# Pixel-Talk/CanonSwap

Measured on AMD Instinct MI355X. Metric: frames/sec at 512x512 (generator hot path F->W->T->R->W->G), higher is better.
Workload: dtype f16; 1 GPU; BASELINE configs[2]: 512x512 video, 64 frames batched per launch on each GPU, steady state over 1280 frames (20 launches per GPU) (256x256 crops in, random-init weights of the real architecture); frames_per_launch_per_gpu=64, frames_total=1280, parallelism=frame-shard x1, identities_resident=1, latency_mode=False, accumulate=fp32, debug_decodes=False

## Files before the change

canonswap_amd/csrc/common.h:

```cpp
#pragma once
#include <hip/hip_runtime.h>
#include <stdint.h>

typedef _Float16 half_t;
typedef _Float16 h8_t __attribute__((ext_vector_type(8)));
typedef _Float16 h4_t __attribute__((ext_vector_type(4)));
typedef float f4_t __attribute__((ext_vector_type(4)));

enum { ACT_NONE = 0, ACT_RELU = 1, ACT_LRELU = 2, ACT_SIGMOID = 3, ACT_GELU = 4 };
enum { MODE_STD = 0, MODE_TBLEND = 1, MODE_SPADE = 2, MODE_PIXSHUF = 3,
       MODE_STDSTAT = 4 };
enum { CFG_128x128 = 0, CFG_128x64 = 1, CFG_256x32 = 2, CFG_256x16 = 3 };
enum { CFG_H_128x128 = 10, CFG_H_128x64 = 11, CFG_H_256x32 = 12, CFG_H_128x32 = 13, CFG_H_128x16 = 14, CFG_H_256x16 = 15,
       CFG_H_SK128x32 = 16 , CFG_H_128x256 = 17,
       CFG_H_128x160 = 18 ,
       CFG_H_256x160 = 19 ,
       CFG_H_256x64 = 20 ,
       CFG_VOL32 = 30 , CFG_WIDE = 31 ,
       CFG_LAT = 32  };

struct TDesc {
    void* p;
    long sN, sD, sH, sW;
};
// ... 45 lines not shown
    int ep_general;
    int pool_hw;
    int spmul;
    const half_t* xs_w; TDesc xs_res, xs_out; int xs_cout;
    int persist_total;
    unsigned in_sample_bytes;
    int nphase;
    long ph_wofs[4];
    unsigned ph_ooff[4];
    int ph_PH[4], ph_PW[4];
    int xf_kind;
    int v32_srows;
    TDesc xf_y, xf_res, xf_out;
    const float* xf_stats; const float* xf_gamma; const float* xf_beta;
    float xf_slope;
#ifdef CS_TIMELINE
    unsigned long long* tl;
    long tl_cap;
#endif
};

__device__ __forceinline__ float gn_scale(float rstd, float gamma) { return rstd * gamma; }
__device__ __forceinline__ float gn_shift(float mean, float sc, float beta) { return fmaf(-mean, sc, beta); }
__device__ __forceinline__ float gn_lrelu(float v, float sc, float sh, float rr, float slope)
{
    float a = fmaf(v, sc, sh);
    a = a + rr;
    return fmaxf(a, a * slope);
}

// ... 15 lines not shown
    long sN, sH, sW;
    const half_t* w1; const half_t* w2;
    const float* b1; const float* b2; const float* s2; const float* t2;
    int act1; float slope1;
    int N, H, W;
};
bool vol32_fused_supported(const ResBlock3dCall& c);
int launch_vol32_fused(const ResBlock3dCall& c, hipStream_t st);
bool vol32_supported(const ConvParams& p);
int vol32_stat_nblk(const ConvParams& p);
int launch_vol32(const ConvParams& p, hipStream_t st);
bool conv_wide_supported(const ConvParams& p, int mode);
int launch_conv_wide(const ConvParams& p, int mode, hipStream_t st);
bool conv_lat_supported(const ConvParams& p, int mode);
int launch_conv_lat(const ConvParams& p, int mode, hipStream_t st);
const half_t* cs_zero_page();

int launch_conv_first(const float* img, const float* w, const float* b, half_t* out, int N, int H, int W, hipStream_t st);
int launch_avgpool(const half_t* in, int N, int D, int H, int W, int C, TDesc out, hipStream_t st);
int launch_dm_compress(const float* f, const float* w, const float* b, half_t* comp, int N, int D, int H, int W, hipStream_t st);
int launch_dm_sparse(const half_t* comp, const float* kp_d, const float* kp_s, half_t* out, int out_stride, int N, int D,
                     int H, int W, hipStream_t st, bool shared_comp = false, bool shared_kps = false);
int launch_dm_softmax(const float* part, const float* bias, const float* kp_d, const float* kp_s, float* deform, float* mask_out,
                      int N, int D, int H, int W, hipStream_t st, int compact = 0, bool shared_kps = false);
int launch_dm_softmax_warp(const float* part, const float* bias, const float* kp_d, const float* kp_s, const float* in, float* out32,
                           half_t* out16, float* deform, int N, int D, int H, int W, hipStream_t st, int compact = 0, bool shared_in = false,
                           bool shared_kps = false);
int launch_occ_finish(const float* part, float bias, float* occ, int N, int H, int W, hipStream_t st);
int launch_occ_finish49(const float* part, float bias, float* occ, int N, int H, int W, hipStream_t st);
int launch_grid_sample(const float* in, const float* grid, float* out32, half_t* out16, int N, int D, int H, int W, hipStream_t st,
// ... 45 lines not shown
```

canonswap_amd/csrc/conv_epilogue.h:

```cpp
#pragma once
#include "common.h"

#ifndef EP_TL
#define EP_TL(i) do { } while (0)
#endif
typedef unsigned int ep_u4_t __attribute__((ext_vector_type(4)));
typedef unsigned int ep_u2_t __attribute__((ext_vector_type(2)));

static inline int ep_check_extents(const ConvParams& p, const char* who)
{
    auto span = [&](const TDesc& t) -> long {
        return (long)(p.N - 1) * t.sN + (long)(p.D - 1) * t.sD + (long)(p.H - 1) * t.sH + (long)(p.W - 1) * t.sW + p.Cout;
    };
    auto wide = [&](const TDesc& t) { return t.sD >= (1L << 23) || t.sH >= (1L << 23) || t.sW >= (1L << 23); };
    const long lim = 1L << 31;
    long ph_max = 0;
    for (int z = 0; z < p.nphase && z < 4; ++z) ph_max = p.ph_ooff[z] > ph_max ? (long)p.ph_ooff[z] : ph_max;
    if ((p.out0.p && span(p.out0) + ph_max >= lim) || (p.out1.p && span(p.out1) >= lim) || (p.res.p && span(p.res) >= lim)) {
        cs_set_error("%s: a tensor of this launch spans 2^31 elements or more (32-bit in-tensor offsets)", who);
        return -1;
    }
    if ((p.out0.p && wide(p.out0)) || (p.out1.p && wide(p.out1)) || (p.res.p && wide(p.res)) || p.D >= (1 << 22) || p.H >= (1 << 22) ||
        p.W >= (1 << 22)) {
        cs_set_error("%s: an axis stride of 2^23 elements or more (24-bit multiplies in the addressing)", who);
// ... 155 lines not shown
            float ep_pa[4], ep_pb[4]; \
_Pragma("unroll") \
            for (int r = 0; r < 4; ++r) { \
                ep_pa[r] = ep_row_sum16(ep_sum[EP_STAT ? ci : 0][r]); ep_pb[r] = ep_row_sum16(ep_sq[EP_STAT ? ci : 0][r]); \
                ep_sum[EP_STAT ? ci : 0][r] = 0.f; ep_sq[EP_STAT ? ci : 0][r] = 0.f; \
            } \
             \
            if (l15 == 0 && cb < p.Cout) { \
                float4* dst = (float4*)(p.stat_out + (((long)tn * ep_nblk + ep_blk) * p.Cout + cb) * 2); \
                dst[0] = make_float4(ep_pa[0], ep_pb[0], ep_pa[1], ep_pb[1]); \
                dst[1] = make_float4(ep_pa[2], ep_pb[2], ep_pa[3], ep_pb[3]); \
            } \
        } \
    }

#ifndef EP_GSEL_V
#define EP_GSEL_V 0
#endif
#ifndef EP_BLK_V
#define EP_BLK_V(sg) ((tile_lin % ep_tiles) * (BM / (EP_SG * 16)) + ep_wpx * (EP_WPX / EP_SG) + (sg))
#define EP_NBLK_V (ep_tiles * (BM / (EP_SG * 16)))
#endif
#ifndef EP_SLICE_FENCE
#define EP_SLICE_FENCE
#endif
#ifndef EP_FG
#define EP_FG 8
#endif
#ifndef EP_FG_F32
#define EP_FG_F32 4
// ... 19 lines not shown
#define EP_O1ONLY_V 0
#endif
#ifndef EP_MLIN_V
#define EP_MLIN_V 0
#endif
#ifndef EP_DUP_V
#define EP_DUP_V 0
#endif
#define EP_SPMULB 256
#define EP_GELUB 512
#define EP_FETCH_ROUND(PG0, BI) \
    if (EP_PF && !EP_EARLY && (ep_fetch || ep_has_ps)) { \
_Pragma("unroll") \
        for (int g = 0; g < EP_G; ++g) { \
            int bw, bh, bd, bn; \
            { int t = (ep_wpx * EP_WPX + (PG0) + g) << 4; bw = t & mW; t >>= lgTW; bh = t & mH; t >>= lgTH; bd = t & mD; t >>= lgTD; bn = t; } \
            if (!EPFAST && ep_nb + ep_ln + bn >= p.N) continue; \
            if (ep_has_ps) ep_ps2[BI][g] = p.pixscale[ep_lane_ps + (unsigned)((((bn * p.D + bd) * p.H + bh) * p.W + bw) * p.ps_stride)]; \
            if (ep_fetch) { \
                const unsigned xb = ep_lane_res + (unsigned)(bn * (int)p.res.sN + bd * (int)p.res.sD + (bh >> ep_rs) * (int)p.res.sH + \
                                                            (bw >> ep_rs) * (int)p.res.sW); \
_Pragma("unroll") \
                for (int ci = 0; ci < WCH; ci += CSTEP) { \
                    const int cb = ep_chan(EP_PAIR, CSTEP, n0 + wch * WCH * 16, ci, l4); \
                    if (!EPALL && cb >= p.Cout) continue; \
                    if (ep_res32) ep_raw2[BI][g][(EP_PF ? ci / CSTEP : 0)] = *(const ep_u4_t*)((const float*)p.res.p + (xb + (unsigned)cb)); \
                    else if (ep_mr && ep_second(EP_PAIR, ci)) {  } \
                    else if (ep_mr && (EPALL || cb + 4 < p.Cout)) ep_raw2[BI][g][(EP_PF ? ci / CSTEP : 0)] = *(const ep_u4_t*)((const half_t*)p.res.p + (xb + (unsigned)cb)); \
                    else { \
                        const ep_u2_t q2 = *(const ep_u2_t*)((const half_t*)p.res.p + (xb + (unsigned)cb)); \
                        ep_raw2[BI][g][(EP_PF ? ci / CSTEP : 0)][0] = q2[0]; ep_raw2[BI][g][(EP_PF ? ci / CSTEP : 0)][1] = q2[1]; \
// ... 79 lines not shown
    ep_u4_t ep_raw2[EP_PIPE ? 2 : 1][EP_G][EP_NCI]; float ep_ps2[EP_PIPE ? 2 : 1][EP_G]; \
    if (EP_PIPE) { EP_FETCH_ROUND(0, 0) } \
_Pragma("unroll") \
    for (int pg = 0; pg < EP_WPX; pg += EP_G) { \
    const int ep_bi = EP_PIPE ? ((pg / EP_G) & 1) : 0; \
    if (!EP_PIPE) { EP_FETCH_ROUND(pg, 0) } \
    else if (pg + EP_G < EP_WPX) { EP_FETCH_ROUND(pg + EP_G, EP_PIPE ? (((pg / EP_G) + 1) & 1) : 0) } \
    ep_u4_t (&ep_raw)[EP_G][EP_NCI] = ep_raw2[ep_bi]; float (&ep_ps)[EP_G] = ep_ps2[ep_bi]; \
    if (pg == 0) EP_TL(6); \
_Pragma("unroll") \
    for (int g = 0; g < EP_G; ++g) { \
        const int pi = pg + g; \
        if (pi == 1) EP_TL(7); \
        if (pi > 0 && pi % EP_SG == 0) { EP_STAT_FLUSH(pi / EP_SG - 1) } \
        int bw, bh, bd, bn; \
        { int t = (ep_wpx * EP_WPX + pi) << 4; bw = t & mW; t >>= lgTW; bh = t & mH; t >>= lgTH; bd = t & mD; t >>= lgTD; bn = t; } \
        if (!EPFAST && ep_nb + ep_ln + bn >= p.N) continue; \
        float ps = 1.f; \
        if (ep_has_ps) ps = EP_PF ? ep_ps[g] : p.pixscale[ep_lane_ps + (unsigned)((((bn * p.D + bd) * p.H + bh) * p.W + bw) * p.ps_stride)]; \
        const unsigned xb = ep_lane_res + (unsigned)(bn * (int)p.res.sN + bd * (int)p.res.sD + (bh >> ep_rs) * (int)p.res.sH + (bw >> ep_rs) * (int)p.res.sW); \
        const unsigned ob0 = ep_lane_o0 + (unsigned)(bn * (int)p.out0.sN + bd * (int)p.out0.sD + (bh >> EP_PS) * (int)p.out0.sH + (bw >> EP_PS) * (int)p.out0.sW); \
        const unsigned ob1 = ep_lane_o1 + (unsigned)(bn * (int)p.out1.sN + bd * (int)p.out1.sD + bh * (int)p.out1.sH + bw * (int)p.out1.sW); \
        float ep_vh[4] = {0.f, 0.f, 0.f, 0.f}, ep_uh[4] = {0.f, 0.f, 0.f, 0.f};       \
_Pragma("unroll") \
        for (int ci = 0; ci < WCH; ci += CSTEP) { \
            const int cb = ep_chan(EP_PAIR, CSTEP, n0 + wch * WCH * 16, ci, l4); \
            if (!EPALL && cb >= p.Cout) continue; \
            float rr[4] = {0.f, 0.f, 0.f, 0.f};      \
            if (ep_has_res) { \
                if (EP_EARLY) { \
                    const h4_t hx = __builtin_bit_cast(h4_t, ep_xpre[EP_EARLY ? pi : 0][EP_EARLY ? ci / 2 : 0]); \
// ... 173 lines not shown
```

canonswap_amd/csrc/conv_halo_kernel.h:

```cpp
#pragma once
#include <type_traits>
#include <utility>
#include <cstdlib>
#include "common.h"
#ifdef CS_TIMELINE
#define EP_TL(i) TL_STAMP(i)
#endif
#define EP_POOL_WSH_V EP_POOL_WSH_K
#define EP_POOL_HSH_V EP_POOL_HSH_K
#define EP_SPMUL_V EP_SPMUL_K
#define EP_DUP_V EP_DUP_K
#define EP_MLIN_V EP_MLIN_K
#define EP_O1ONLY_V EP_O1ONLY_K
#define EP_O0_EXTRA_V ep_o0_extra
#include "conv_epilogue.h"

typedef unsigned int u4_t __attribute__((ext_vector_type(4)));
__device__ __forceinline__ unsigned mdiv(unsigned u, unsigned magic) { return magic ? __umulhi(u, magic) : u; }

template <int OFF>
__device__ __forceinline__ void wfrag_load(u4_t& dst, const half_t* ptr)
{
    asm volatile("global_load_dwordx4 %0, %1, off offset:%2" : "=v"(dst) : "v"(ptr), "n"(OFF));
}
template <int N>
__device__ __forceinline__ void wait_vmcnt_le()
{
    asm volatile("s_waitcnt vmcnt(%0)" ::"n"(N) : "memory");
}
// ... 45 lines not shown
    if (PAD == 2) return ST == 3 ? 16 : (ST == 9 ? 19 : ((ST == 7 || ST == 8) ? 15 : (ST == 16 ? 13 : 8)));
    return ST == 4 ? 18 : ((ST == 3 || ST == 7 || ST == 8 || ST == 9) ? 13 : (ST == 12 ? 9 : 8));
}
template <int ST, int PAD> __host__ __device__ constexpr int halo_lane_pos(int l)
{
#ifdef CS_LDS_V1
    return l;
#else
    using SS = StaticShape<ST>;
    if (ST == 0 || SS::KW != 3 || SS::LW > 3 || SS::LW < 2) return l;
    if (SS::LW == 2 && PAD == 2) return ((l & 1) << 1) | ((l & 2) << 2) | ((l >> 2) & 1) | ((l & 8) >> 1);
    return ((l & 1) << 1) | ((l & 2) << 1) | ((l >> 2) & 1) | (l & 8);
#endif
}

template <class F, int... I> __device__ __forceinline__ void halo_static_for_impl(F&& f, std::integer_sequence<int, I...>) { (f(std::integral_constant<int, I>{}), ...); }
template <int N, class F> __device__ __forceinline__ void halo_static_for(F&& f) { halo_static_for_impl(static_cast<F&&>(f), std::make_integer_sequence<int, N>{}); }

template <int WCH, int PFS, int HI, int ST0>
constexpr int halo_ring_young(int st, int L, int NP, bool dma_cur)
{
    auto dma = [&](int u, bool on) { return (on && u >= ST0 && u < ST0 + HI) ? 1 : 0; };
    auto cur_before = [&](int from_step ) {
        int n = 0;
        for (int u = from_step; u < st; ++u) n += (u >= 1 ? WCH : 0) + dma(u, dma_cur);
        return n;
    };
    if (st >= PFS) {
        const int u0 = st - PFS + 1;
        return dma(u0, dma_cur) + cur_before(u0 + 1);
// ... 35 lines not shown
    constexpr int SLP = SL + PAD;
    constexpr bool EP_POOLK = ST != 0 && !SK && MODE == MODE_STD && WCH == 2 && SS::KD == 3 && SS::KH == 3 && SS::KW == 3 && (SS::LW == 3 || SS::LW == 2) && SS::LH >= 1;
    constexpr bool EP_POOLK2 = halo_pool2d<CK, WPX, WCH, WVP, MODE, SK, ST>();
    constexpr bool XSK = ST == 1 && !SK && MODE == MODE_STD && CK == 64 && WCH == 4 && WPX == 8 && WVP == 1;
#ifdef CS_NO_SPMUL_FAST
    constexpr bool EP_SPMUL_K = false;
#else
    constexpr bool EP_SPMUL_K = ST == 1 && !SK && MODE == MODE_STD && CK == 64 && WCH == 4 && WPX == 8 && WVP == 1;
#endif
    constexpr bool EP_O1ONLY_K = ST == 16 && !SK && MODE == MODE_STD;
    constexpr bool EP_MLIN_K = ST == 15 && !SK && MODE == MODE_STD;
    constexpr bool EP_DUP_K = (ST == 11 || ST == 14 || ST == 15) && !SK && MODE == MODE_STD && WCH == 2 && WPX == 8;
    constexpr int EP_POOL_WSH_K = EP_POOLK ? halo_pool_shift<ST, PAD>(0) : (EP_POOLK2 ? 1 : 0);
    constexpr int EP_POOL_HSH_K = EP_POOLK ? halo_pool_shift<ST, PAD>(SS::LW) : 0;
    constexpr int VS = SLP * 16;
    constexpr int HI = halo_hi<ST, PAD>();
    constexpr int KH32 = CK / 32;
    constexpr int PFD = 4;
    constexpr int SKS = SK ? 4 : 1;
    static_assert(WVP * WVC == 4, "4 waves per workgroup");
    static_assert(!SK || (WVC == 1 && WPX == 8), "split-K variants: every wave covers all 128 positions");

    extern __shared__ __attribute__((aligned(16))) unsigned char smem[];
#ifdef CS_TIMELINE
    unsigned long long tl_t[8] = {0, 0, 0, 0, 0, 0, 0, 0};
    const unsigned long long tl_real0 = __builtin_amdgcn_s_memrealtime();
    TL_STAMP(0);
#endif

#ifdef CS_DEPHASE
// ... 124 lines not shown
            for (int q0 = 0; q0 < nitems; q0 += 256) {
                const int q = q0 + tid;
                if (q < nitems) {
                    bool inb;
                    const int o = piece_off(q, inb);
                    const bool ok = inb && ((q % SLP) * 8 < climit);
                    glds(ok ? p.in + o + coff : p.zero, buf, q0 + wave * 64);
                }
            }
        }
    };

    int abase[WPX];
#pragma unroll
    for (int pi = 0; pi < WPX; ++pi) {
        int m = wpx * WPX * 16 + pi * 16 + l15p;
        const int wl = m & mW; m >>= lgTW;
        const int hl = m & mH; m >>= lgTH;
        const int dl = m & mD; m >>= lgTD;
        abase[pi] = (((m * HD + dl) * HH + hl) * HW + wl) * VS + l4 * 16;
    }
    const int nck = (p.Cin + CK - 1) / CK;
    const int j0 = SK ? wave : 0;
    int cc_lo = 0, cc_hi = nck;
    if (p.sk_out) { cc_lo = (int)(((long)nck * blockIdx.z) / gridDim.z); cc_hi = (int)(((long)nck * (blockIdx.z + 1)) / gridDim.z); }

    const half_t* wbase = p.wgt;
    if (p.wslot) wbase += p.wofs[p.wslot[nb < p.N ? nb : p.N - 1]];
    if (PHK && p.nphase) wbase += p.ph_wofs[phz];
    const half_t* wlane = wbase + ((long)(n0 + wch * WCH * 16) * 32 + ep_lane_row(EP_PAIR, l15) * 32 + l4 * 8);
    const long wstep = (long)p.Cout_pad * 32;

#ifdef CS_NO_EARLY
    constexpr bool EP_EARLY = false;
#else
    constexpr bool EP_EARLY = (MODE == MODE_SPADE) && !SK && ST != 0 && WCH == 2 && WPX == 8;
#endif
#ifdef CS_NO_EPFAST
    constexpr bool EP_FAST = false;
#else
    constexpr bool EP_FAST = !SK && ST != 0 && (WCH == 4 || WCH == 5 || (WCH == 2 && WPX == 8) || ST == 15);
#endif
    constexpr int EP_WPX0 = WPX;
    const int ep_wpx0 = wpx;
    CONV_EPILOGUE_EARLY_FETCH()

    f4_t acc[WCH][WPX];
#pragma unroll
    for (int ci = 0; ci < WCH; ++ci)
#pragma unroll
        for (int pi = 0; pi < WPX; ++pi) acc[ci][pi] = (f4_t){0.f, 0.f, 0.f, 0.f};

    if constexpr (ST != 0) {
        constexpr int NT = SS::KD * SS::KH * SS::KW, NS = NT * KH32;
        constexpr bool RAGK = (CK == 32) && (WPX == 8) && (ST == 7 || ST == 8 || ST == 9) && MODE == MODE_STD;
        constexpr bool LATK = CK == 64 && WCH == 2 && WPX == 4 && ST == 1 && !SK;
#ifdef CS_PFS3
        constexpr int PFS = NS < 3 ? NS : 3;
#else
// ... 9 lines not shown
#endif
#endif
        constexpr int SHW = (1 << SS::LW) + SS::KW - 1, SHH = (1 << SS::LH) + SS::KH - 1;
#ifdef CS_NO_ASMRING
        constexpr bool ASMR = false;
#else
        constexpr bool ASMR = DB && WCH == 5 && WPX == 8 && WVP == 2 && (ST == 7 || ST == 8 || ST == 9) && MODE == MODE_STD && PFS == 3;
#endif
        if constexpr (ASMR) {
            static_assert(SK == false && KH32 == 1, "ASMR: 32-channel chunks");
            constexpr int HSTRIDE = HI * 4096;
            constexpr int ST0 = 1;
            constexpr unsigned OOB = 0x80000000u;
            static_assert(ASMRK, "the kernel-level and the block-level conditions of ASMR agree");
            auto (&wr) = wr_p;
            auto set_stage = [&](int n_, int d0_, int h0_, int w0_) {
                rsrc_p = __builtin_amdgcn_make_buffer_rsrc((void*)(p.in + (long)n_ * p.in_sN), 0, (int)p.in_sample_bytes, 0x00020000);
                int tid_o = tid;
                asm volatile("" : "+v"(tid_o));
#pragma unroll
                for (int j = 0; j < HI; ++j) {
                    const int q = tid_o + 256 * j;
                    const int hv = q / SLP, sl = q % SLP;
                    const int hw = hv % HW; int r = hv / HW;
                    const int hh = r % HH; r /= HH;
                    const int id = d0_ + r - p.PD, ih = h0_ + hh - PHv, iw = w0_ + hw - PWv;
                    const bool inb = q < nitems && sl < SL && r < HD && (unsigned)id < (unsigned)p.D && (unsigned)ih < (unsigned)p.H && (unsigned)iw < (unsigned)p.W;
                    poffb[j] = inb ? (unsigned)(__mul24(id, isD) + __mul24(ih >> p.up_shift, isH) + __mul24(iw >> p.up_shift, isW) + sl * 8) * 2u : OOB;
                }
            };
            auto stage_piece = [&](int buf, int cn, int j) {
// ... 13 lines not shown
            auto wload1 = [&](u4_t& dst, const half_t* src, int ci) {
                if (ci == 0) asm volatile("global_load_dwordx4 %0, %1, off" : "=v"(dst) : "v"(src));
                else if (ci == 1) asm volatile("global_load_dwordx4 %0, %1, off offset:1024" : "=v"(dst) : "v"(src));
                else if (ci == 2) asm volatile("global_load_dwordx4 %0, %1, off offset:2048" : "=v"(dst) : "v"(src));
                else if (ci == 3) asm volatile("global_load_dwordx4 %0, %1, off offset:3072" : "=v"(dst) : "v"(src));
                else asm volatile("global_load_dwordx4 %0, %1, off" : "=v"(dst) : "v"(src + 4 * 16 * 32));
            };
            static_assert(EP_PAIR == 0, "ASMR: plain weight row order");
            TL_STAMP(1);
            constexpr bool CARRY = ST != 9;
            if (!staged) {
                set_stage(nb, d0, h0, w0);
#pragma unroll
                for (int j = 0; j < HI; ++j) stage_piece(gbuf, cc_lo, j);
            }
            if (!staged || !CARRY) {
#pragma unroll
                for (int st = 0; st < PFS; ++st)
#pragma unroll
                    for (int ci = 0; ci < WCH; ++ci) wload1(wr[st][ci], wsrc_of(cc_lo, st, NS), ci);
            }
            TL_STAMP(2);
            auto run_chunk_a = [&](int cc, auto rag_t) {
                constexpr bool RAG = decltype(rag_t)::value;
                wait_vmcnt_le<PFS * WCH>();
                __builtin_amdgcn_s_barrier();
                asm volatile("" ::: "memory");
                const unsigned char* hb = smem + (size_t)gbuf * HSTRIDE;
                const int nbuf = gbuf ^ 1;
                gbuf ^= 1;
                if (cc + 1 == cc_hi && has_next) {
                    int ntl, ncb_, t2 = 0, q2;
                    u_to_tile(p_base + p_i + p_per * (p_j + 1), ntl, ncb_);
                    t2 = ntl;
                    q2 = (int)mdiv((unsigned)t2, p.mg_tw); const int tw2 = t2 - q2 * p.nTW; t2 = q2;
                    q2 = (int)mdiv((unsigned)t2, p.mg_th); const int th2 = t2 - q2 * p.nTH; t2 = q2;
                    q2 = (int)mdiv((unsigned)t2, p.mg_td); const int td2 = t2 - q2 * p.nTD; t2 = q2;
                    set_stage(t2 * TN, td2 << lgTD, th2 << lgTH, tw2 << lgTW);
                }
// ... 1 lines not shown
                constexpr int PK = SS::KW > 1 ? SS::KW : SS::KH, SPR = PK / 2 + PK % 2;
                constexpr int NSC = RAG ? (NT / PK) * SPR : NS;
                auto tap_of = [&](int st) -> int { return RAG ? (st / SPR) * PK + 2 * (st % SPR) : st; };
                auto paired = [&](int st) -> bool { return RAG && (st % SPR) < PK / 2; };
                auto toff_of = [&](int st) -> int {
                    const int tap = tap_of(st);
                    return (((tap / (SS::KW * SS::KH)) * SHH + (tap / SS::KW) % SS::KH) * SHW + tap % SS::KW) * VS;
                };
                int abP[RAG ? WPX : 1];
                if constexpr (RAG) {
                    const int pd = (l4 >= 2) ? (SS::KW > 1 ? VS : SHW * VS) - 32 : 0;
#pragma unroll
                    for (int pi = 0; pi < WPX; ++pi) abP[pi] = abase[pi] + pd;
                }
                auto ab_of = [&](int pi, int st) -> int { return paired(st) ? abP[RAG ? pi : 0] : abase[pi]; };
                h8_t afA[HA], afB[WPX - HA];
#pragma unroll
                for (int pi = 0; pi < HA; ++pi) afA[pi] = *(const h8_t*)(hb + ab_of(pi, 0) + toff_of(0));
                halo_static_for<NSC>([&](auto stc) {
                    constexpr int st = decltype(stc)::value;
                    {
#ifdef CS_ASMR_DEBUG0
                        constexpr int NY = 0;
#else
                        constexpr int NY = halo_ring_young<WCH, PFS, HI, ST0>(st, NSC, NS, true);
#endif
                        asm volatile("s_waitcnt vmcnt(%5)" : "+v"(wr[st % PFS][0]), "+v"(wr[st % PFS][1]), "+v"(wr[st % PFS][2]), "+v"(wr[st % PFS][3]),
                                                             "+v"(wr[st % PFS][4]) : "n"(NY));
                    }
                    __builtin_amdgcn_sched_barrier(0);
                    const half_t* rsrc_w = wsrc_of(cc, st - 1 + PFS, NSC);
                    const int toff = toff_of(st);
#pragma unroll
                    for (int k = 0; k < 2 * WCH; ++k) {
                        const int ci = k >> 1, p0 = (k & 1) * 2;
                        acc[ci][p0] = __builtin_amdgcn_mfma_f32_16x16x32_f16(__builtin_bit_cast(h8_t, wr[st % PFS][ci]), afA[p0], acc[ci][p0], 0, 0, 0);
                        acc[ci][p0 + 1] = __builtin_amdgcn_mfma_f32_16x16x32_f16(__builtin_bit_cast(h8_t, wr[st % PFS][ci]), afA[p0 + 1], acc[ci][p0 + 1], 0, 0, 0);
                        if (k >= 2 && k < 6) afB[k - 2] = *(const h8_t*)(hb + ab_of(HA + k - 2, st) + toff);
                        if constexpr (st >= 1) { if (k >= 5) wload1(wr[(st - 1) % PFS][k - 5], rsrc_w, k - 5); }
                        __builtin_amdgcn_sched_barrier(0);
                    }
                    if (st >= ST0 && st < ST0 + HI) { stage_piece(nbuf, cc + 1, st - ST0); __builtin_amdgcn_sched_barrier(0); }
#pragma unroll
                    for (int k = 0; k < 2 * WCH; ++k) {
                        const int ci = k >> 1, p0 = (k & 1) * 2;
                        acc[ci][HA + p0] = __builtin_amdgcn_mfma_f32_16x16x32_f16(__builtin_bit_cast(h8_t, wr[st % PFS][ci]), afB[p0], acc[ci][HA + p0], 0, 0, 0);
                        acc[ci][HA + p0 + 1] = __builtin_amdgcn_mfma_f32_16x16x32_f16(__builtin_bit_cast(h8_t, wr[st % PFS][ci]), afB[p0 + 1], acc[ci][HA + p0 + 1], 0, 0, 0);
                        if (k >= 2 && k < 6 && st + 1 < NSC) afA[k - 2] = *(const h8_t*)(hb + ab_of(k - 2, st + 1) + toff_of(st + 1));
                        __builtin_amdgcn_sched_barrier(0);
                    }
                });
                {
                    const half_t* rsrc_w = wsrc_of(cc, NSC - 1 + PFS, NSC);
#pragma unroll
                    for (int ci = 0; ci < WCH; ++ci) wload1(wr[(NSC - 1) % PFS][ci], rsrc_w, ci);
                }
            };
            const bool rag = RAGK && p.ragged && cc_hi == nck;
            for (int cc = cc_lo; cc < cc_hi - (rag ? 1 : 0); ++cc) run_chunk_a(cc, std::false_type{});
            if constexpr (RAGK) {
                if (rag) run_chunk_a(cc_hi - 1, std::true_type{});
            }
            staged = has_next;
            if (!has_next || !CARRY) {
                wait_vmcnt_le<0>();
                __builtin_amdgcn_sched_barrier(0);
            }
#pragma unroll
            for (int st = 0; st < PFS; ++st)
                asm volatile("" :: "v"(wr[st][0]), "v"(wr[st][1]), "v"(wr[st][2]), "v"(wr[st][3]), "v"(wr[st][4]));
        } else {
        u4_t wr[PFS][WCH];
        auto wload_at = [&](u4_t (&dst)[WCH], int cc, int st) {
            const int ccl = cc < nck ? cc : nck - 1;
            const half_t* src = wlane + (long)((ccl * KH32 + st % KH32) * NT + st / KH32) * wstep;
#pragma unroll
            for (int ci = 0; ci < WCH; ++ci) dst[ci] = *(const u4_t*)(src + ep_frag_row(EP_PAIR, ci) * 32);
        };
        TL_STAMP(1);
        stage_halo(0, cc_lo * CK);
        __syncthreads();
        TL_STAMP(2);
        if (DB && cc_lo + 1 < cc_hi) stage_halo(1, (cc_lo + 1) * CK);
        auto chunk_head = [&](int cc) -> const unsigned char* {
            if (!WCARRY || cc == cc_lo) {
// ... 182 lines not shown
    }

    if constexpr (ST == 0) {
        wait_vmcnt_le<0>();
        __builtin_amdgcn_sched_barrier(0);
    }

    constexpr bool EP_HEAVY = (MODE == MODE_PIXSHUF) || (WCH == 1) || (ST == 15) || (ST == 0);
    constexpr bool KWSUM = !SK && MODE == MODE_STD && WCH == 5 && WPX == 8 && WVP == 2 && (ST == 8 || ST == 9);
    TL_STAMP(3);
    if constexpr (!SK) {
        if (p.sk_out) {
            const long mtot = (long)p.N * p.D * p.H * p.W;
#pragma unroll
            for (int pi = 0; pi < WPX; ++pi) {
                int m = wpx * WPX * 16 + pi * 16 + l15p;
                const int w = (tw << lgTW) + (m & mW); m >>= lgTW;
                const int h = (th << lgTH) + (m & mH); m >>= lgTH;
                const int d = (td << lgTD) + (m & mD); m >>= lgTD;
                const int n = tn * TN + m;
                if (n >= p.N) continue;
                const long pos = (((long)n * p.D + d) * p.H + h) * p.W + w;
#pragma unroll
                for (int ci = 0; ci < WCH; ++ci)
                    *(f4_t*)(p.sk_out + ((long)blockIdx.z * mtot + pos) * p.Cout_pad + ep_chan(EP_PAIR, 1, n0 + wch * WCH * 16, ci, l4)) = acc[ci][pi];
            }
        } else if (XSK && p.xs_w) {
            if constexpr (XSK) {
                __syncthreads();
                float* part = (float*)smem;
                const int cw0 = n0 + wch * 64;
// ... 94 lines not shown
                    const int fi = q * 128 + th128;
                    on[q] = fi < 220;
                    const int fic = on[q] ? fi : 0;
                    goff[q] = (fic / 55) * (p.nTW * 220) + (fic % 55) * 4;
#pragma unroll
                    for (int e = 0; e < 4; ++e) {
                        const int idx = (fic % 55) * 4 + e, c = idx % 22, j = idx / 22, h = fic / 55;
#pragma unroll
                        for (int t = 0; t < 4; ++t) {
                            const int kw = t + 6 - j;
                            offT[q][e][t] = (kw >= 0 && kw <= 6) ? ((h << 2) | t) * 160 + kw * 22 + c : ZERO;
                        }
                    }
                }
                const long gslice = (long)p.H * p.nTW * 220;
                float* const gbase = p.kw_out + ((((long)tn * p.D + (td << lgTD) + wpx * 4) * p.H + (th << lgTH)) * p.nTW + tw) * 220;
#pragma unroll
                for (int pi = 0; pi < WPX; ++pi) {
#pragma unroll
                    for (int ci = 0; ci < WCH; ++ci) *(f4_t*)(buf + l15p * 160 + wch * (WCH * 16) + ci * 16 + l4 * 4) = acc[ci][pi];
                    __syncthreads();
#pragma unroll
                    for (int q = 0; q < 2; ++q) {
                        if (on[q]) {
                            f4_t v;
#pragma unroll
                            for (int e = 0; e < 4; ++e) v[e] = ((buf[offT[q][e][0]] + buf[offT[q][e][1]]) + buf[offT[q][e][2]]) + buf[offT[q][e][3]];
                            *(f4_t*)(gbase + (pi >> 1) * gslice + (long)(pi & 1) * 4 * (p.nTW * 220) + goff[q]) = v;
                        }
                    }
                    __syncthreads();
                }
            } else if constexpr (KWSUM) {
                __syncthreads();
                constexpr int ZERO = 16 * 160;
                float* buf = (float*)(smem + (ASMRK ? (size_t)(gbuf ^ 1) * (HI * 4096) : 0)) + wpx * (16 * 160 + 4);
                const int th128 = wch * 64 + lane;
                if (th128 == 0) buf[ZERO] = 0.f;
                int offA[12], offB[12], goff[3];
#pragma unroll
                for (int q = 0; q < 3; ++q) {
                    const int fi = q * 128 + th128;
                    goff[q] = (fi * 4 / 176) * (p.nTW * 176) + (fi * 4) % 176;
// ... 166 lines not shown
    constexpr bool asmr = false;
#endif
    const bool db = nck > 1 && (asmr ? 2 * HI * 4096 <= 160 * 1024 : 2 * HV * VS <= (big || (WCH == 4 && PAD == 2) ? 128 : 64) * 1024) && HV * SLP <= 256 * HI;
    size_t lds = (size_t)(db ? 2 : 1) * HV * VS + 16;
    ConvParams kp = p;
    if (asmr && db) {
        lds = (size_t)2 * HI * 4096;
        const long span = (long)(p.inD - 1) * p.in_sD + (long)((p.H - 1) >> p.up_shift) * p.in_sH + (long)((p.W - 1) >> p.up_shift) * p.in_sW + p.Cin + 32;
        if (span >= (1L << 30) || p.cg > 0 || p.hilo || (1 << lgS) != BM) {
            cs_set_error("conv_halo: the 256 x 160 tiles address one sample of the input through a buffer of less than 2^31 bytes (no grouped / split-precision input)");
            return -1;
        }
        kp.in_sample_bytes = (unsigned)(span * 2);
    }
    kp.persist_total = 0;
    if (SK && lds < (size_t)4 * WCH * WPX * 4 * 64 * sizeof(float)) lds = (size_t)4 * WCH * WPX * 4 * 64 * sizeof(float);
    if (p.xs_w && lds < (size_t)32768) lds = 32768;
    if (lds > 160 * 1024) { cs_set_error("conv_halo: halo of %ld voxels does not fit LDS", HV); return -1; }
    dim3 grid((unsigned)(p.nTW * p.nTH * p.nTD * p.nTN), (unsigned)(p.Cout_pad / BN));
    if (p.hilo && (ST == 0 || CK != 32 || nck != 3 || db || p.sk_out)) {
        cs_set_error("conv_halo: the hi/lo split-precision mode needs a static-shape 32-channel kernel with three single-buffered chunks");
        return -1;
    }
    if (p.nphase) {
        if (SK || !halo_phase_group<WCH, ST>() || p.nphase < 1 || p.nphase > 4 || p.sk_out || p.kw_out || p.xs_w || p.persist_total < 0) { cs_set_error("conv_halo: bad grouped launch (%d phases)", p.nphase); return -1; }
        if (p.res.p || p.stat_out || p.pixscale || p.spmul || p.pool_hw) { cs_set_error("conv_halo: a grouped launch carries out0 / out1 only (no res / statistics / pixel scale / spmul / pooling)"); return -1; }
        for (int z = 0; z < p.nphase; ++z)
            if (p.ph_ooff[z] % 8u) { cs_set_error("conv_halo: output offset of phase %d (%u elements) is not a multiple of 8 (16-byte stores)", z, p.ph_ooff[z]); return -1; }
        grid.z = (unsigned)p.nphase;
    }
// ... 45 lines not shown
```

canonswap_amd/csrc/engine.hip:

```cpp
#include "common.h"
#include "../../include/canonswap_hip.h"

#include <cstdarg>
#include <cstdio>
#include <cstdlib>
#include <cstring>
#include <initializer_list>
#include <map>
#include <string>
#include <vector>

static thread_local char g_err[1024] = "";
void cs_set_error(const char* fmt, ...)
{
    va_list ap;
    va_start(ap, fmt);
    vsnprintf(g_err, sizeof(g_err), fmt, ap);
    va_end(ap);
}
extern "C" const char* cs_last_error(void) { return g_err; }
extern "C" int cs_abi_version(void) { return CS_ABI_VERSION; }

#define TRY(x) do { if ((x) != 0) return -1; } while (0)

// ... 105 lines not shown
    {
        void* q = nullptr;
        hipError_t e = hipMalloc(&q, n * sizeof(T));
        if (e != hipSuccess) { cs_set_error("hipMalloc(%zu bytes): %s", n * sizeof(T), hipGetErrorString(e)); return -1; }
        allocs.push_back(q);
        *p = (T*)q;
        return 0;
    }
    const Blob* find(const std::string& n) const
    {
        auto it = blobs.find(n);
        return it == blobs.end() ? nullptr : &it->second;
    }
};

namespace {

int need(cs_engine* e, const std::string& n, size_t bytes, const void** out)
{
    const Blob* b = e->find(n);
    if (!b) { cs_set_error("weights: blob '%s' was not uploaded", n.c_str()); return -1; }
    if (bytes && b->bytes != bytes) { cs_set_error("weights: blob '%s' has %zu bytes, expected %zu", n.c_str(), b->bytes, bytes); return -1; }
    *out = b->p;
    return 0;
}

int get_conv(cs_engine* e, const std::string& n, int Cin, int Cout_pad, int Cout, int KD, int KH, int KW, int bias_len,
             double macs, ConvL* L)
{
    const int nch = (Cin + 31) / 32;
// ... 102 lines not shown
    if (Cout_pad % 32 == 0) return CFG_H_128x32;
    return CFG_H_128x16;
}

int amax_after(cs_engine* e, const struct ConvCall& c, hipStream_t st);

constexpr int VOL32_MINB = 3;
bool vol32_enabled() { static const bool on = [] { const char* s = getenv("CANONSWAP_VOL32"); return !s || atoi(s) != 0; }(); return on; }
bool vol32_xf() { static const bool on = [] { const char* s = getenv("CANONSWAP_VOL32_XF"); return !s || atoi(s) != 0; }(); return on && vol32_enabled(); }

int go(cs_engine* e, ConvCall& c, hipStream_t st, int prefW = 0, int prefH = 0)
{
    const int nph = c.p.nphase > 0 ? c.p.nphase : 1;
    const double fl = 2.0 * c.macs_per_pos * (double)c.p.N * c.p.D * c.p.H * c.p.W * nph;
    e->flops += fl;
    {
        double ksteps = (double)c.p.nchunks * c.p.KD * c.p.KH * c.p.KW;
        if (c.p.ragged) {
            const int NT = c.p.KD * c.p.KH * c.p.KW, PK = c.p.KW > 1 ? c.p.KW : c.p.KH;
            ksteps -= NT - (NT / PK) * (PK / 2 + PK % 2);
        }
        e->flops_exec += 2.0 * (double)c.p.N * c.p.D * c.p.H * c.p.W * c.p.Cout_pad * 32.0 * ksteps * nph;
    }
    if (vol32_enabled() && vol32_supported(c.p) && (c.p.N >= VOL32_MINB || c.p.stat_out || c.p.xf_kind)) {
        if (e->latency_mode && c.p.stat_out) c.p.v32_srows = 2;
        c.stat_nblk = vol32_stat_nblk(c.p);
        TRY(e->run(0, st, [&] { return launch_vol32(c.p, st); }, c.name, fl));
        return amax_after(e, c, st);
    }
    if (c.p.xf_kind) { cs_set_error("%s: transform staging needs the vol32 kernel", c.name); return -1; }
    static const int wide_on = [] { const char* s = getenv("CANONSWAP_WIDE"); return s ? atoi(s) : 1; }();
    if (wide_on && !e->latency_mode && c.hcfg < 0 && (c.mode != MODE_SPADE || wide_on >= 2)) {
        if (conv_wide_supported(c.p, c.mode) && (long)c.p.N * (c.p.H / 16) * (c.p.W / 16) * (c.p.Cout_pad / 256) >= 512) {
            c.stat_nblk = (c.p.W / 16) * (c.p.H / 8) * 2;
            TRY(e->run(0, st, [&] { return launch_conv_wide(c.p, c.mode, st); }, c.name, fl));
            return amax_after(e, c, st);
        }
    }
    if (e->latency_mode && c.hcfg < 0 && conv_lat_supported(c.p, c.mode) &&
        (long)c.p.N * (c.p.H / 8) * (c.p.W / 16) * (c.p.Cout_pad / (c.mode == MODE_TBLEND ? 128 : 64)) <= 256) {
        c.stat_nblk = (c.p.W / 16) * (c.p.H / 8) * 2;
        TRY(e->run(0, st, [&] { return launch_conv_lat(c.p, c.mode, st); }, c.name, fl));
        return amax_after(e, c, st);
    }
    if (c.p.inD == c.p.D) {
        const int hcfg = c.hcfg >= 0 ? c.hcfg : pick_halo_cfg(c.p, c.mode);
        const int BM = (hcfg == CFG_H_256x32 || hcfg == CFG_H_256x16 || hcfg == CFG_H_256x160 || hcfg == CFG_H_256x64) ? 256 : 128;
        const bool is3d = c.p.KD > 1;
        if (!prefW) { prefW = is3d ? 8 : 16; prefH = is3d ? 8 : BM / 16; }
        set_tile(c.p, BM, prefW, prefH);
        {
            int wave_px = 64;
            if (hcfg == CFG_H_128x32 || hcfg == CFG_H_128x16 || hcfg == CFG_H_SK128x32) wave_px = 32;
            c.stat_nblk = c.p.nTW * c.p.nTH * c.p.nTD * (BM / wave_px);
        }
        const bool spade_ck32 = c.mode == MODE_SPADE && c.p.Cout_pad % 256 != 0;
        const bool k11 = c.p.KD == 1 && c.p.KH == 1 && c.p.KW == 1;
        const bool cg64 = c.cg_ck64 && k11 && c.p.cg > 0 && !(c.p.cg & 1) && c.p.Cin % 64 == 0 && c.mode == MODE_STD;
        const int ck = (!is3d && c.p.Cin % 64 == 0 && (c.p.cg == 0 || cg64) && !spade_ck32) ? 64 : 32;
        c.p.xcd_map = XCD_MAP;
        c.p.persist_total = HALO_PERSIST;
        {
            const bool sk_on = e->latency_mode;
            const int bn = hcfg == CFG_H_128x256 ? 256 : hcfg == CFG_H_128x128 ? 128 : hcfg == CFG_H_128x64 || hcfg == CFG_H_256x64 ? 64 :
                           hcfg == CFG_H_128x160 || hcfg == CFG_H_256x160 ? 160 : hcfg == CFG_H_128x16 || hcfg == CFG_H_256x16 ? 16 : 32;
// ... 1472 lines not shown
```

Baseline: 550.5 frames/s.

## Skip dead depth-padding taps in depth-major halo conv tiles at volume edges

Adds a depth-major block order for one halo conv configuration (ST 9, WCH 5, WPX 8, WVP 2). In tiles at the first or last depth slab, MFMAs and LDS fragment loads whose depth tap falls entirely in zero padding are skipped. The tile body is specialized per edge type, and weight ring priming and draining move inside that body. The kw-sum output addressing and epilogue block indexing are remapped to the new order, and the flop accounting is adjusted. The main risks are more code size and register pressure from three instantiations, and possible changes to access locality from the new block order.

```diff
diff --git a/canonswap_amd/csrc/common.h b/canonswap_amd/csrc/common.h
--- a/canonswap_amd/csrc/common.h
+++ b/canonswap_amd/csrc/common.h
@@ -83,6 +83,7 @@
     TDesc xf_y, xf_res, xf_out;
     const float* xf_stats; const float* xf_gamma; const float* xf_beta;
     float xf_slope;
+    int dskip;
 #ifdef CS_TIMELINE
     unsigned long long* tl;
     long tl_cap;
@@ -128,6 +129,7 @@
 int launch_conv_wide(const ConvParams& p, int mode, hipStream_t st);
 bool conv_lat_supported(const ConvParams& p, int mode);
 int launch_conv_lat(const ConvParams& p, int mode, hipStream_t st);
+bool halo_mask_dskip();
 const half_t* cs_zero_page();
 
 int launch_conv_first(const float* img, const float* w, const float* b, half_t* out, int N, int H, int W, hipStream_t st);
diff --git a/canonswap_amd/csrc/conv_epilogue.h b/canonswap_amd/csrc/conv_epilogue.h
--- a/canonswap_amd/csrc/conv_epilogue.h
+++ b/canonswap_amd/csrc/conv_epilogue.h
@@ -193,6 +193,9 @@
         } \
     }
 
+#ifndef EP_BLKIDX_V
+#define EP_BLKIDX_V(pi) (ep_wpx * EP_WPX + (pi))
+#endif
 #ifndef EP_GSEL_V
 #define EP_GSEL_V 0
 #endif
@@ -242,7 +245,7 @@
 _Pragma("unroll") \
         for (int g = 0; g < EP_G; ++g) { \
             int bw, bh, bd, bn; \
-            { int t = (ep_wpx * EP_WPX + (PG0) + g) << 4; bw = t & mW; t >>= lgTW; bh = t & mH; t >>= lgTH; bd = t & mD; t >>= lgTD; bn = t; } \
+            { int t = EP_BLKIDX_V((PG0) + g) << 4; bw = t & mW; t >>= lgTW; bh = t & mH; t >>= lgTH; bd = t & mD; t >>= lgTD; bn = t; } \
             if (!EPFAST && ep_nb + ep_ln + bn >= p.N) continue; \
             if (ep_has_ps) ep_ps2[BI][g] = p.pixscale[ep_lane_ps + (unsigned)((((bn * p.D + bd) * p.H + bh) * p.W + bw) * p.ps_stride)]; \
             if (ep_fetch) { \
@@ -352,7 +355,7 @@
         if (pi == 1) EP_TL(7); \
         if (pi > 0 && pi % EP_SG == 0) { EP_STAT_FLUSH(pi / EP_SG - 1) } \
         int bw, bh, bd, bn; \
-        { int t = (ep_wpx * EP_WPX + pi) << 4; bw = t & mW; t >>= lgTW; bh = t & mH; t >>= lgTH; bd = t & mD; t >>= lgTD; bn = t; } \
+        { int t = EP_BLKIDX_V(pi) << 4; bw = t & mW; t >>= lgTW; bh = t & mH; t >>= lgTH; bd = t & mD; t >>= lgTD; bn = t; } \
         if (!EPFAST && ep_nb + ep_ln + bn >= p.N) continue; \
         float ps = 1.f; \
         if (ep_has_ps) ps = EP_PF ? ep_ps[g] : p.pixscale[ep_lane_ps + (unsigned)((((bn * p.D + bd) * p.H + bh) * p.W + bw) * p.ps_stride)]; \
diff --git a/canonswap_amd/csrc/conv_halo_kernel.h b/canonswap_amd/csrc/conv_halo_kernel.h
--- a/canonswap_amd/csrc/conv_halo_kernel.h
+++ b/canonswap_amd/csrc/conv_halo_kernel.h
@@ -13,6 +13,8 @@
 #define EP_MLIN_V EP_MLIN_K
 #define EP_O1ONLY_V EP_O1ONLY_K
 #define EP_O0_EXTRA_V ep_o0_extra
+#define EP_BLKIDX_V(pi) (DMAJ ? (pi) * WVP + ep_wpx : ep_wpx * EP_WPX + (pi))
+#define HALO_BLK_POS(pi) (DMAJ ? ((pi) * WVP + wpx) * 16 : wpx * WPX * 16 + (pi) * 16)
 #include "conv_epilogue.h"
 
 typedef unsigned int u4_t __attribute__((ext_vector_type(4)));
@@ -88,6 +90,12 @@
 #endif
 }
 
+template <int ST, int WCH, int WPX, int WVP, bool SK> constexpr bool halo_depth_major() { return ST == 9 && WCH == 5 && WPX == 8 && WVP == 2 && !SK; }
+template <int EDGE> __host__ __device__ constexpr bool halo_dlive(int pi, int kd, int PD, int TD)
+{
+    return EDGE == 1 ? pi + kd >= PD : (EDGE == 2 ? pi + kd < TD + PD : true);
+}
+
 template <class F, int... I> __device__ __forceinline__ void halo_static_for_impl(F&& f, std::integer_sequence<int, I...>) { (f(std::integral_constant<int, I>{}), ...); }
 template <int N, class F> __device__ __forceinline__ void halo_static_for(F&& f) { halo_static_for_impl(static_cast<F&&>(f), std::make_integer_sequence<int, N>{}); }
 
@@ -153,6 +161,7 @@
     constexpr int EP_POOL_WSH_K = EP_POOLK ? halo_pool_shift<ST, PAD>(0) : (EP_POOLK2 ? 1 : 0);
     constexpr int EP_POOL_HSH_K = EP_POOLK ? halo_pool_shift<ST, PAD>(SS::LW) : 0;
     constexpr int VS = SLP * 16;
+    constexpr bool DMAJ = halo_depth_major<ST, WCH, WPX, WVP, SK>();
     constexpr int HI = halo_hi<ST, PAD>();
     constexpr int KH32 = CK / 32;
     constexpr int PFD = 4;
@@ -307,7 +316,7 @@
     int abase[WPX];
 #pragma unroll
     for (int pi = 0; pi < WPX; ++pi) {
-        int m = wpx * WPX * 16 + pi * 16 + l15p;
+        int m = HALO_BLK_POS(pi) + l15p;
         const int wl = m & mW; m >>= lgTW;
         const int hl = m & mH; m >>= lgTH;
         const int dl = m & mD; m >>= lgTD;
@@ -336,6 +345,7 @@
 #endif
     constexpr int EP_WPX0 = WPX;
     const int ep_wpx0 = wpx;
+    static_assert(!(EP_EARLY && DMAJ), "the early fetch walks consecutive blocks");
     CONV_EPILOGUE_EARLY_FETCH()
 
     f4_t acc[WCH][WPX];
@@ -375,7 +385,7 @@
             constexpr unsigned OOB = 0x80000000u;
             static_assert(ASMRK, "the kernel-level and the block-level conditions of ASMR agree");
             auto (&wr) = wr_p;
-            auto set_stage = [&](int n_, int d0_, int h0_, int w0_) {
+            auto set_stage = [&](int n_, int d0_, int h0_, int w0_) __attribute__((always_inline)) {
                 rsrc_p = __builtin_amdgcn_make_buffer_rsrc((void*)(p.in + (long)n_ * p.in_sN), 0, (int)p.in_sample_bytes, 0x00020000);
                 int tid_o = tid;
                 asm volatile("" : "+v"(tid_o));
@@ -419,6 +429,8 @@
 #pragma unroll
                 for (int j = 0; j < HI; ++j) stage_piece(gbuf, cc_lo, j);
             }
+            static_assert(!(DMAJ && CARRY), "the depth-major tile primes and drains its ring inside the body it picks (run_tile)");
+            if constexpr (!DMAJ) {
             if (!staged || !CARRY) {
 #pragma unroll
                 for (int st = 0; st < PFS; ++st)
@@ -426,8 +438,11 @@
                     for (int ci = 0; ci < WCH; ++ci) wload1(wr[st][ci], wsrc_of(cc_lo, st, NS), ci);
             }
             TL_STAMP(2);
-            auto run_chunk_a = [&](int cc, auto rag_t) {
+            }
+            auto run_chunk_a = [&](int cc, auto rag_t, auto edge_t) {
                 constexpr bool RAG = decltype(rag_t)::value;
+                constexpr int EDGE = decltype(edge_t)::value;
+                static_assert(EDGE == 0 || DMAJ, "dead depth taps are a property of a whole fragment in the depth-major tile only");
                 wait_vmcnt_le<PFS * WCH>();
                 __builtin_amdgcn_s_barrier();
                 asm volatile("" ::: "memory");
@@ -459,9 +474,10 @@
                     for (int pi = 0; pi < WPX; ++pi) abP[pi] = abase[pi] + pd;
                 }
                 auto ab_of = [&](int pi, int st) -> int { return paired(st) ? abP[RAG ? pi : 0] : abase[pi]; };
+                auto live = [&](int pi, int st) -> bool { return EDGE == 0 || halo_dlive<EDGE>(pi, tap_of(st) / (SS::KW * SS::KH), SS::KD / 2, 1 << SS::LD); };
                 h8_t afA[HA], afB[WPX - HA];
 #pragma unroll
-                for (int pi = 0; pi < HA; ++pi) afA[pi] = *(const h8_t*)(hb + ab_of(pi, 0) + toff_of(0));
+                for (int pi = 0; pi < HA; ++pi) if (live(pi, 0)) afA[pi] = *(const h8_t*)(hb + ab_of(pi, 0) + toff_of(0));
                 halo_static_for<NSC>([&](auto stc) {
                     constexpr int st = decltype(stc)::value;
                     {
@@ -479,9 +495,9 @@
 #pragma unroll
                     for (int k = 0; k < 2 * WCH; ++k) {
                         const int ci = k >> 1, p0 = (k & 1) * 2;
-                        acc[ci][p0] = __builtin_amdgcn_mfma_f32_16x16x32_f16(__builtin_bit_cast(h8_t, wr[st % PFS][ci]), afA[p0], acc[ci][p0], 0, 0, 0);
-                        acc[ci][p0 + 1] = __builtin_amdgcn_mfma_f32_16x16x32_f16(__builtin_bit_cast(h8_t, wr[st % PFS][ci]), afA[p0 + 1], acc[ci][p0 + 1], 0, 0, 0);
-                        if (k >= 2 && k < 6) afB[k - 2] = *(const h8_t*)(hb + ab_of(HA + k - 2, st) + toff);
+                        if (live(p0, st)) acc[ci][p0] = __builtin_amdgcn_mfma_f32_16x16x32_f16(__builtin_bit_cast(h8_t, wr[st % PFS][ci]), afA[p0], acc[ci][p0], 0, 0, 0);
+                        if (live(p0 + 1, st)) acc[ci][p0 + 1] = __builtin_amdgcn_mfma_f32_16x16x32_f16(__builtin_bit_cast(h8_t, wr[st % PFS][ci]), afA[p0 + 1], acc[ci][p0 + 1], 0, 0, 0);
+                        if (k >= 2 && k < 6 && live(HA + k - 2, st)) afB[k - 2] = *(const h8_t*)(hb + ab_of(HA + k - 2, st) + toff);
                         if constexpr (st >= 1) { if (k >= 5) wload1(wr[(st - 1) % PFS][k - 5], rsrc_w, k - 5); }
                         __builtin_amdgcn_sched_barrier(0);
                     }
@@ -489,9 +505,9 @@
 #pragma unroll
                     for (int k = 0; k < 2 * WCH; ++k) {
                         const int ci = k >> 1, p0 = (k & 1) * 2;
-                        acc[ci][HA + p0] = __builtin_amdgcn_mfma_f32_16x16x32_f16(__builtin_bit_cast(h8_t, wr[st % PFS][ci]), afB[p0], acc[ci][HA + p0], 0, 0, 0);
-                        acc[ci][HA + p0 + 1] = __builtin_amdgcn_mfma_f32_16x16x32_f16(__builtin_bit_cast(h8_t, wr[st % PFS][ci]), afB[p0 + 1], acc[ci][HA + p0 + 1], 0, 0, 0);
-                        if (k >= 2 && k < 6 && st + 1 < NSC) afA[k - 2] = *(const h8_t*)(hb + ab_of(k - 2, st + 1) + toff_of(st + 1));
+                        if (live(HA + p0, st)) acc[ci][HA + p0] = __builtin_amdgcn_mfma_f32_16x16x32_f16(__builtin_bit_cast(h8_t, wr[st % PFS][ci]), afB[p0], acc[ci][HA + p0], 0, 0, 0);
+                        if (live(HA + p0 + 1, st)) acc[ci][HA + p0 + 1] = __builtin_amdgcn_mfma_f32_16x16x32_f16(__builtin_bit_cast(h8_t, wr[st % PFS][ci]), afB[p0 + 1], acc[ci][HA + p0 + 1], 0, 0, 0);
+                        if (k >= 2 && k < 6 && st + 1 < NSC && live(k - 2, st + 1)) afA[k - 2] = *(const h8_t*)(hb + ab_of(k - 2, st + 1) + toff_of(st + 1));
                         __builtin_amdgcn_sched_barrier(0);
                     }
                 });
@@ -502,11 +518,33 @@
                 }
             };
             const bool rag = RAGK && p.ragged && cc_hi == nck;
-            for (int cc = cc_lo; cc < cc_hi - (rag ? 1 : 0); ++cc) run_chunk_a(cc, std::false_type{});
+            if constexpr (DMAJ) {
+                auto run_tile = [&](auto edge_t) __attribute__((always_inline)) {
+#pragma unroll
+                    for (int st = 0; st < PFS; ++st)
+#pragma unroll
+                        for (int ci = 0; ci < WCH; ++ci) wload1(wr[st][ci], wsrc_of(cc_lo, st, NS), ci);
+                    TL_STAMP(2);
+                    for (int cc = cc_lo; cc < cc_hi - (rag ? 1 : 0); ++cc) run_chunk_a(cc, std::false_type{}, edge_t);
+                    if (rag) run_chunk_a(cc_hi - 1, std::true_type{}, edge_t);
+                    wait_vmcnt_le<0>();
+                    __builtin_amdgcn_sched_barrier(0);
+#pragma unroll
+                    for (int st = 0; st < PFS; ++st)
+                        asm volatile("" :: "v"(wr[st][0]), "v"(wr[st][1]), "v"(wr[st][2]), "v"(wr[st][3]), "v"(wr[st][4]));
+                };
+                const int edge = !p.dskip ? 0 : (d0 == 0 ? 1 : (d0 + (1 << SS::LD) >= p.D ? 2 : 0));
+                if (edge == 1) run_tile(std::integral_constant<int, 1>{});
+                else if (edge == 2) run_tile(std::integral_constant<int, 2>{});
+                else run_tile(std::integral_constant<int, 0>{});
+            } else {
+            for (int cc = cc_lo; cc < cc_hi - (rag ? 1 : 0); ++cc) run_chunk_a(cc, std::false_type{}, std::integral_constant<int, 0>{});
             if constexpr (RAGK) {
-                if (rag) run_chunk_a(cc_hi - 1, std::true_type{});
+                if (rag) run_chunk_a(cc_hi - 1, std::true_type{}, std::integral_constant<int, 0>{});
+            }
             }
             staged = has_next;
+            if constexpr (!DMAJ) {
             if (!has_next || !CARRY) {
                 wait_vmcnt_le<0>();
                 __builtin_amdgcn_sched_barrier(0);
@@ -514,6 +552,7 @@
 #pragma unroll
             for (int st = 0; st < PFS; ++st)
                 asm volatile("" :: "v"(wr[st][0]), "v"(wr[st][1]), "v"(wr[st][2]), "v"(wr[st][3]), "v"(wr[st][4]));
+            }
         } else {
         u4_t wr[PFS][WCH];
         auto wload_at = [&](u4_t (&dst)[WCH], int cc, int st) {
@@ -726,7 +765,7 @@
             const long mtot = (long)p.N * p.D * p.H * p.W;
 #pragma unroll
             for (int pi = 0; pi < WPX; ++pi) {
-                int m = wpx * WPX * 16 + pi * 16 + l15p;
+                int m = HALO_BLK_POS(pi) + l15p;
                 const int w = (tw << lgTW) + (m & mW); m >>= lgTW;
                 const int h = (th << lgTH) + (m & mH); m >>= lgTH;
                 const int d = (td << lgTD) + (m & mD); m >>= lgTD;
@@ -851,7 +890,8 @@
                     }
                 }
                 const long gslice = (long)p.H * p.nTW * 220;
-                float* const gbase = p.kw_out + ((((long)tn * p.D + (td << lgTD) + wpx * 4) * p.H + (th << lgTH)) * p.nTW + tw) * 220;
+                static_assert(DMAJ, "the 4-column kw sum follows the depth-major block order");
+                float* const gbase = p.kw_out + ((((long)tn * p.D + (td << lgTD)) * p.H + (th << lgTH) + wpx * 4) * p.nTW + tw) * 220;
 #pragma unroll
                 for (int pi = 0; pi < WPX; ++pi) {
 #pragma unroll
@@ -863,7 +903,7 @@
                             f4_t v;
 #pragma unroll
                             for (int e = 0; e < 4; ++e) v[e] = ((buf[offT[q][e][0]] + buf[offT[q][e][1]]) + buf[offT[q][e][2]]) + buf[offT[q][e][3]];
-                            *(f4_t*)(gbase + (pi >> 1) * gslice + (long)(pi & 1) * 4 * (p.nTW * 220) + goff[q]) = v;
+                            *(f4_t*)(gbase + pi * gslice + goff[q]) = v;
                         }
                     }
                     __syncthreads();
@@ -1060,6 +1100,7 @@
         kp.in_sample_bytes = (unsigned)(span * 2);
     }
     kp.persist_total = 0;
+    kp.dskip = (halo_depth_major<ST, WCH, WPX, WVP, SK>() && asmr && db && p.PD == p.KD / 2 && halo_mask_dskip()) ? 1 : 0;
     if (SK && lds < (size_t)4 * WCH * WPX * 4 * 64 * sizeof(float)) lds = (size_t)4 * WCH * WPX * 4 * 64 * sizeof(float);
     if (p.xs_w && lds < (size_t)32768) lds = 32768;
     if (lds > 160 * 1024) { cs_set_error("conv_halo: halo of %ld voxels does not fit LDS", HV); return -1; }
diff --git a/canonswap_amd/csrc/engine.hip b/canonswap_amd/csrc/engine.hip
--- a/canonswap_amd/csrc/engine.hip
+++ b/canonswap_amd/csrc/engine.hip
@@ -143,6 +143,8 @@
     }
 };
 
+bool halo_mask_dskip() { static const bool on = [] { const char* s = getenv("CANONSWAP_MASK_DSKIP"); return !s || atoi(s) != 0; }(); return on; }
+
 namespace {
 
 int need(cs_engine* e, const std::string& n, size_t bytes, const void** out)
@@ -275,13 +277,15 @@
     const int nph = c.p.nphase > 0 ? c.p.nphase : 1;
     const double fl = 2.0 * c.macs_per_pos * (double)c.p.N * c.p.D * c.p.H * c.p.W * nph;
     e->flops += fl;
+    double fl_exec = 0;
     {
         double ksteps = (double)c.p.nchunks * c.p.KD * c.p.KH * c.p.KW;
         if (c.p.ragged) {
             const int NT = c.p.KD * c.p.KH * c.p.KW, PK = c.p.KW > 1 ? c.p.KW : c.p.KH;
             ksteps -= NT - (NT / PK) * (PK / 2 + PK % 2);
         }
-        e->flops_exec += 2.0 * (double)c.p.N * c.p.D * c.p.H * c.p.W * c.p.Cout_pad * 32.0 * ksteps * nph;
+        fl_exec = 2.0 * (double)c.p.N * c.p.D * c.p.H * c.p.W * c.p.Cout_pad * 32.0 * ksteps * nph;
+        e->flops_exec += fl_exec;
     }
     if (vol32_enabled() && vol32_supported(c.p) && (c.p.N >= VOL32_MINB || c.p.stat_out || c.p.xf_kind)) {
         if (e->latency_mode && c.p.stat_out) c.p.v32_srows = 2;
@@ -310,6 +314,8 @@
         const bool is3d = c.p.KD > 1;
         if (!prefW) { prefW = is3d ? 8 : 16; prefH = is3d ? 8 : BM / 16; }
         set_tile(c.p, BM, prefW, prefH);
+        if (hcfg == CFG_H_256x160 && c.p.KD == 7 && c.p.PD == 3 && c.p.lgTW == 2 && c.p.lgTD == 3 && c.p.D % 8 == 0 && c.p.nchunks > 1 && halo_mask_dskip())
+            e->flops_exec -= fl_exec * (c.p.nTD > 1 ? 12.0 : 6.0) / (7.0 * c.p.D);
         {
             int wave_px = 64;
             if (hcfg == CFG_H_128x32 || hcfg == CFG_H_128x16 || hcfg == CFG_H_SK128x32) wave_px = 32;
```

Result: no change. 552.2 frames/s, median of 6 (+0.3%).
